# zhaoyuhsin/Edge-Guided-Near-Eye-Image-Analysis-for-Head-Mounted-Displays

Measured on AMD Instinct MI355X. Metric: eye-frames/sec (320x240): inference edge+seg (value), +fit, exact fp32, and train fwd+bwd at 1 MI355X, higher is better.
Workload: dtype f32 tensors; inference products split into f16 hi/lo pairs (3 f16 MFMAs per product, 22-bit significand), f32 accumulate (`exact_fp32`: every product on the f32 MFMA); `train`: bf16 storage, f32 accumulate, f32 master weights (and an f32-storage leg)

## Files before the change

edge-guided-near-eye-image-analysis-for-head-mounted-displays_amd/csrc/conv1x1_f16.hip:

```cpp
#include "common.h"
#include "split_f16.h"

typedef float f32x16 __attribute__((ext_vector_type(16)));
typedef float f32x4 __attribute__((ext_vector_type(4)));
typedef float f32x2 __attribute__((ext_vector_type(2)));
typedef _Float16 h8 __attribute__((ext_vector_type(8)));
typedef _Float16 h2 __attribute__((ext_vector_type(2)));
typedef unsigned u32x4 __attribute__((ext_vector_type(4)));

namespace {

constexpr unsigned OOB = 0x80000000u;

__device__ __forceinline__ __amdgpu_buffer_rsrc_t make_rsrc(const void* base, unsigned bytes) {
  return __builtin_amdgcn_make_buffer_rsrc(const_cast<void*>(base), 0, (int)bytes, 0x00020000);
}

__device__ __forceinline__ void split8(const u32x4 a, const u32x4 b, float s, h8& hi, h8& lo) {
  const f32x4 va = __builtin_bit_cast(f32x4, a), vb = __builtin_bit_cast(f32x4, b);
  const float x[8] = {va[0], va[1], va[2], va[3], vb[0], vb[1], vb[2], vb[3]};
#pragma unroll
  for (int q = 0; q < 4; ++q) {
    h2 h, l;
    egne::split2(x[2 * q], x[2 * q + 1], s, h, l);
// ... 73 lines not shown
    }
    const __amdgpu_buffer_rsrc_t ro = make_rsrc(p.out + m0 * p.out_pix_stride, (unsigned)(rows * p.out_pix_stride * 4));
    bool bad = false;
    [[maybe_unused]] int o00 = 0, o01 = 0, o10 = 0, o11 = 0;
    [[maybe_unused]] float w00 = 0.f, w01 = 0.f, w10 = 0.f, w11 = 0.f;
    [[maybe_unused]] __amdgpu_buffer_rsrc_t rres = ro;
    [[maybe_unused]] bool pix_ok = false, staged = false;
    if constexpr (UP) {
      const int ph = p.Ho, pw = p.Wo, hw = p.H * p.W;
      const long long m = m0 + li;
      pix_ok = m < M;
      const int b = pix_ok ? (int)(m / hw) : 0;
      const int r = pix_ok ? (int)(m - (long long)b * hw) : 0;
      const int y = r / p.W, x = r - y * p.W;
      float sy = 0.5f * (y + 0.5f) - 0.5f, sx = 0.5f * (x + 0.5f) - 0.5f;
      sy = sy < 0.f ? 0.f : sy; sx = sx < 0.f ? 0.f : sx;
      const int y0 = (int)sy, x0 = (int)sx, y1 = y0 + (y0 < ph - 1 ? 1 : 0), x1 = x0 + (x0 < pw - 1 ? 1 : 0);
      const float ly = sy - y0, lx = sx - x0;
      w00 = (1.f - ly) * (1.f - lx); w01 = (1.f - ly) * lx; w10 = ly * (1.f - lx); w11 = ly * lx;
      const int rs = (int)p.res_pix_stride, base = b * ph * pw;
      rres = make_rsrc(p.residual, (unsigned)((long long)p.B * ph * pw * rs * 4));
      const int r0 = (int)(m0 % hw), xb0 = r0 % p.W;
      staged = rows == 32 && xb0 + 32 <= p.W;
      if (staged) {
        const int bb = (int)(m0 / hw), yb = r0 / p.W;
        float syb = 0.5f * (yb + 0.5f) - 0.5f; syb = syb < 0.f ? 0.f : syb;
        const int yb0 = (int)syb, yb1 = yb0 + (yb0 < ph - 1 ? 1 : 0);
        const float lyb = syb - yb0;
        float sxb = 0.5f * (xb0 + 0.5f) - 0.5f; sxb = sxb < 0.f ? 0.f : sxb;
        const int cb = (int)sxb;
        constexpr int VPP = 8 * TN;
        for (int it = lane; it < UPC * VPP; it += 64) {
          const int cc = it / VPP, c4 = it - cc * VPP;
          const int gx = cb + cc < pw ? cb + cc : pw - 1;
          const int n = nt0 * 32 + c4 * 4;
          const int o0 = n < p.Cout_store ? (((bb * ph + yb0) * pw + gx) * rs + p.res_ch_off + n) * 4 : (int)OOB;
          const int o1 = n < p.Cout_store ? (((bb * ph + yb1) * pw + gx) * rs + p.res_ch_off + n) * 4 : (int)OOB;
          const f32x4 ra = __builtin_bit_cast(f32x4, __builtin_amdgcn_raw_buffer_load_b128(rres, o0, 0, 0));
          const f32x4 rb = __builtin_bit_cast(f32x4, __builtin_amdgcn_raw_buffer_load_b128(rres, o1, 0, 0));
          *(f32x4*)&patch[cc * UPP + c4 * 4] = (1.f - lyb) * ra + lyb * rb;
        }
        asm volatile("s_waitcnt vmcnt(0) lgkmcnt(0)" ::: "memory");
        o00 = ((x0 - cb) * UPP) * 4; o01 = ((x1 - cb) * UPP) * 4;
        w00 = 1.f - lx; w01 = lx;
      } else {
        o00 = ((base + y0 * pw + x0) * rs + p.res_ch_off) * 4; o01 = ((base + y0 * pw + x1) * rs + p.res_ch_off) * 4;
        o10 = ((base + y1 * pw + x0) * rs + p.res_ch_off) * 4; o11 = ((base + y1 * pw + x1) * rs + p.res_ch_off) * 4;
      }
    }
#pragma unroll
    for (int tn = 0; tn < TN; ++tn)
#pragma unroll
      for (int j = 0; j < 4; ++j) {
        const int n = (nt0 + tn) * 32 + 8 * j + 4 * kq;
        f32x4 v;
#pragma unroll
        for (int e = 0; e < 4; ++e) {
          const float t = acc[tn][4 * j + e] * out_scale + bias[tn][j][e];
          v[e] = fmaxf(t, t * slope);
        }
        if (tn == 0 && j == 0) bad |= egne_nonfinite(v[0]);
        if constexpr (UP) {
          if (staged) {
            const char* pb = (const char*)patch + (tn * 32 + 8 * j + 4 * kq) * 4;
            v += w00 * *(const f32x4*)(pb + o00) + w01 * *(const f32x4*)(pb + o01);
          } else {
          const bool on = pix_ok && n < p.Cout_store;
          const f32x4 a = __builtin_bit_cast(f32x4, __builtin_amdgcn_raw_buffer_load_b128(rres, on ? o00 + n * 4 : (int)OOB, 0, 0));
          const f32x4 b_ = __builtin_bit_cast(f32x4, __builtin_amdgcn_raw_buffer_load_b128(rres, on ? o01 + n * 4 : (int)OOB, 0, 0));
          const f32x4 c = __builtin_bit_cast(f32x4, __builtin_amdgcn_raw_buffer_load_b128(rres, on ? o10 + n * 4 : (int)OOB, 0, 0));
          const f32x4 d_ = __builtin_bit_cast(f32x4, __builtin_amdgcn_raw_buffer_load_b128(rres, on ? o11 + n * 4 : (int)OOB, 0, 0));
          v += w00 * a + w01 * b_ + w10 * c + w11 * d_;
          }
        }
        const int off = n < p.Cout_store ? (li * (int)p.out_pix_stride + p.out_ch_off + n) * 4 : (int)OOB;
        __builtin_amdgcn_raw_buffer_store_b128(__builtin_bit_cast(u32x4, v), ro, off, 0, 0);
      }
    egne_ovf_commit(bad, p.ovf_flag);
  }
}


template <int TN, bool STATS = false>
__global__ __launch_bounds__(256) void conv1x1_pool_f16x3_kernel(const egne_conv_desc p, const _Float16* __restrict__ fhi,
                                                                 const _Float16* __restrict__ flo, float a_scale, float out_scale,
                                                                 int G, long long M, int nblocks) {
  extern __shared__ __attribute__((aligned(16))) _Float16 wl[];
  const int tid = threadIdx.x, lane = tid & 63, wave = tid >> 6;
  const int li = lane & 31, kq = lane >> 5;
  const int NT = p.CoutP >> 5, nt0 = blockIdx.y * TN;
  for (int it = tid; it < G * TN * 2 * 64; it += 256) {
    const int l = it & 63, hl = (it >> 6) & 1;
    const int tn = (it >> 7) % TN, g = (it >> 7) / TN;
    const _Float16* src = (hl ? flo : fhi) + (((long long)g * NT + nt0 + tn) * 64 + l) * 8;
    *(u32x4*)&wl[(long long)it * 8] = *(const u32x4*)src;
  }
  __syncthreads();

  const float slope = p.act == EGNE_ACT_RELU ? 0.f : (p.act == EGNE_ACT_LEAKY ? 0.01f : 1.f);
  [[maybe_unused]] f32x4 bias[STATS ? 1 : TN][4];
  if constexpr (!STATS) {
#pragma unroll
  for (int tn = 0; tn < TN; ++tn)
#pragma unroll
    for (int j = 0; j < 4; ++j) {
      const int n = (nt0 + tn) * 32 + 8 * j + 4 * kq;
      bias[tn][j] = (p.bias && n < p.Cout_store) ? *(const f32x4*)(p.bias + n) : (f32x4)(0.f);
    }
  }
  const int H = p.H, W = p.W, Hp = p.Ho, Wp = p.Wo, hwp = Hp * Wp;
  const float s4 = 0.25f * a_scale;

  constexpr bool stats = STATS;
  const int bpf = (hwp + 31) >> 5, cb = stats ? (bpf + p.stats_nchunk - 1) / p.stats_nchunk : 1;
  constexpr int PP = 36;
  [[maybe_unused]] float* const patch = (float*)(wl + (long long)G * TN * 2 * 64 * 8) + wave * (32 * PP);
  [[maybe_unused]] const int rd = (lane >> 5) * PP + (lane & 31);

  for (int unit = blockIdx.x * 4 + wave; unit < nblocks; unit += gridDim.x * 4) {
   long long mfirst = (long long)unit * 32, mend = M;
   if (stats) {
     const int fb = unit / p.stats_nchunk, ck = unit - fb * p.stats_nchunk;
     mfirst = (long long)fb * hwp + (long long)ck * cb * 32;
     mend = (long long)(fb + 1) * hwp;
   }
   if (mend > mfirst + (long long)cb * 32) mend = mfirst + (long long)cb * 32;
   [[maybe_unused]] double ssum[TN], qsum[TN];
#pragma unroll
   for (int tn = 0; tn < TN; ++tn) ssum[tn] = qsum[tn] = 0.;
   for (long long m0 = mfirst; m0 < mend; m0 += 32) {
    const long long rows = mend - m0 < 32 ? mend - m0 : 32;
    const int b0 = (int)(m0 / hwp);
    const long long m = m0 + li;
    const bool valid = li < rows;
    const int b = valid ? (int)(m / hwp) : b0;
    const int r = (int)(m - (long long)b * hwp);
    const int yp = valid ? r / Wp : 0, xp = valid ? r - yp * Wp : 0;
    const int pin = ((b - b0) * H + 2 * yp) * W + 2 * xp;
    f32x16 acc[TN];
#pragma unroll
    for (int tn = 0; tn < TN; ++tn) acc[tn] = (f32x16)(0.f);
    int g = 0;
    for (int s = 0; s < p.nseg; ++s) {
      const egne_seg sg = p.seg[s];
      const long long frame = (long long)H * W * sg.pix_stride;
      const long long left = ((long long)p.B - b0) * frame * 4;
      const __amdgpu_buffer_rsrc_t rs = make_rsrc(sg.ptr + (long long)b0 * frame, (unsigned)(left < 2 * frame * 4 ? left : 2 * frame * 4));
      const int ps4 = (int)sg.pix_stride * 4;
      const int voff = valid ? (pin * (int)sg.pix_stride + sg.ch_off + 4 * kq) * 4 : (int)OOB;
      const float slope_in = sg.act_in == EGNE_ACT_RELU ? 0.f : (sg.act_in == EGNE_ACT_LEAKY ? 0.01f : 1.f);
      const float* tsc = sg.scale + (long long)b * sg.Cp + 4 * kq;
      const float* tsh = sg.shift + (long long)b * sg.Cp + 4 * kq;
      const int n16 = (sg.Cp + 15) >> 4;
      const bool tail8 = (sg.Cp & 15) != 0;
      for (int gg = 0; gg < n16; ++gg) {
        const bool has_b = !(tail8 && gg == n16 - 1);
        const int ob = has_b ? voff + 32 : (int)OOB;
        u32x4 xa[4], xb[4];
#pragma unroll
        for (int t = 0; t < 4; ++t) {
          const int d = ((t >> 1) * W + (t & 1)) * ps4;
          xa[t] = __builtin_amdgcn_raw_buffer_load_b128(rs, voff == (int)OOB ? (int)OOB : voff + d, gg * 64, 0);
          xb[t] = __builtin_amdgcn_raw_buffer_load_b128(rs, ob == (int)OOB ? (int)OOB : ob + d, gg * 64, 0);
        }
        const f32x4 sca = *(const f32x4*)(tsc + gg * 16), sha = *(const f32x4*)(tsh + gg * 16);
        const f32x4 scb = has_b ? *(const f32x4*)(tsc + gg * 16 + 8) : (f32x4)(0.f), shb = has_b ? *(const f32x4*)(tsh + gg * 16 + 8) : (f32x4)(0.f);
        f32x4 sa = (f32x4)(0.f), sb = (f32x4)(0.f);
#pragma unroll
        for (int t = 0; t < 4; ++t) {
          f32x4 va = __builtin_bit_cast(f32x4, xa[t]) * sca + sha, vb = __builtin_bit_cast(f32x4, xb[t]) * scb + shb;
#pragma unroll
          for (int e = 0; e < 4; ++e) { sa[e] += fmaxf(va[e], va[e] * slope_in); sb[e] += fmaxf(vb[e], vb[e] * slope_in); }
        }
        if (!valid) { sa = (f32x4)(0.f); sb = (f32x4)(0.f); }
        h8 ah, al;
        split8(__builtin_bit_cast(u32x4, sa), __builtin_bit_cast(u32x4, sb), s4, ah, al);
        const _Float16* wp = wl + ((long long)(g + gg) * TN * 2 * 64 + lane) * 8;
#pragma unroll
        for (int tn = 0; tn < TN; ++tn) {
          const h8 wh = *(const h8*)(wp + (tn * 2 + 0) * 512), wo = *(const h8*)(wp + (tn * 2 + 1) * 512);
          acc[tn] = __builtin_amdgcn_mfma_f32_32x32x16_f16(wh, al, acc[tn], 0, 0, 0);
          acc[tn] = __builtin_amdgcn_mfma_f32_32x32x16_f16(wo, ah, acc[tn], 0, 0, 0);
          acc[tn] = __builtin_amdgcn_mfma_f32_32x32x16_f16(wh, ah, acc[tn], 0, 0, 0);
        }
      }
      g += n16;
    }
    const __amdgpu_buffer_rsrc_t ro = make_rsrc(p.out + m0 * p.out_pix_stride, (unsigned)(rows * p.out_pix_stride * 4));
    bool bad = false;
#pragma unroll
    for (int tn = 0; tn < TN; ++tn)
#pragma unroll
      for (int j = 0; j < 4; ++j) {
        const int n = (nt0 + tn) * 32 + 8 * j + 4 * kq;
        f32x4 v, bv;
        if constexpr (STATS) bv = (p.bias && n < p.Cout_store) ? *(const f32x4*)(p.bias + n) : (f32x4)(0.f);
        else bv = bias[tn][j];
#pragma unroll
        for (int e = 0; e < 4; ++e) {
          const float t = acc[tn][4 * j + e] * out_scale + bv[e];
          v[e] = fmaxf(t, t * slope);
        }
        if (tn == 0 && j == 0) bad |= egne_nonfinite(v[0]);
        const int off = n < p.Cout_store ? (li * (int)p.out_pix_stride + p.out_ch_off + n) * 4 : (int)OOB;
        __builtin_amdgcn_raw_buffer_store_b128(__builtin_bit_cast(u32x4, v), ro, off, 0, 0);
        if constexpr (stats) {
          *(f32x4*)&patch[li * PP + 8 * j + 4 * kq] = valid ? v : (f32x4)(0.f);
          if (j == 3) {
            asm volatile("s_waitcnt lgkmcnt(0)" ::: "memory");
            double s_ = ssum[tn], q_ = qsum[tn];
#pragma unroll
            for (int i = 0; i < 16; ++i) {
              const double x = (double)patch[i * 2 * PP + rd];
              s_ += x; q_ += x * x;
            }
            ssum[tn] = s_; qsum[tn] = q_;
          }
        }
      }
    egne_ovf_commit(bad, p.ovf_flag);
   }
   if constexpr (stats) {
#pragma unroll
     for (int tn = 0; tn < TN; ++tn) {
       const double s_ = ssum[tn] + __shfl_xor(ssum[tn], 32), q_ = qsum[tn] + __shfl_xor(qsum[tn], 32);
       const int n = (nt0 + tn) * 32 + lane;
       if (lane < 32 && n < p.Cout_store)
         ((double2*)p.stats_ws)[(long long)unit * p.Cout_store + n] = make_double2(s_, q_);
     }
   }
  }
}

__global__ void pack_w1x1_f16_k(const float* __restrict__ w, int Cout, int Cin, const int* __restrict__ kmap, int G, int CoutP,
                                float wscale, _Float16* __restrict__ hi, _Float16* __restrict__ lo) {
  const long long total = (long long)G * CoutP * 16;
  const int NT = CoutP >> 5;
  for (long long i = (long long)blockIdx.x * blockDim.x + threadIdx.x; i < total; i += (long long)gridDim.x * blockDim.x) {
    const int j = (int)(i & 7), nn = (int)((i >> 3) & 31), h = (int)((i >> 8) & 1);
    long long q = i >> 9;
    const int nt = (int)(q % NT);
    const int g = (int)(q / NT);
    const int n = nt * 32 + nn, ci = kmap[g * 16 + h * 8 + j];
    const float v = (n < Cout && ci >= 0) ? w[(long long)n * Cin + ci] * wscale : 0.f;
    const _Float16 hh = (_Float16)v;
    hi[i] = hh;
    lo[i] = (_Float16)(v - (float)hh);
  }
}

}

extern "C" int egne_pack_conv1x1_weight_f16(const float* w_oihw, int Cout, int Cin, const int32_t* kmap, int G, int CoutP,
                                            float wscale, void* fhi, void* flo, void* stream) {
  EGNE_REQUIRE(w_oihw && kmap && fhi && flo && Cout > 0 && Cin > 0 && G > 0 && CoutP >= Cout && CoutP % 32 == 0 && wscale > 0.f,
               "pack_conv1x1_f16: bad sizes Cout %d Cin %d G %d CoutP %d", Cout, Cin, G, CoutP);
  long long total = (long long)G * CoutP * 16, g = (total + 255) / 256;
  if (g > 4096) g = 4096;
  hipLaunchKernelGGL(pack_w1x1_f16_k, dim3((unsigned)g), dim3(256), 0, (hipStream_t)stream, w_oihw, Cout, Cin, kmap, G, CoutP, wscale,
                     (_Float16*)fhi, (_Float16*)flo);
  return egne::check_launch("egne_pack_conv1x1_weight_f16");
}

extern "C" int egne_conv1x1_f16x3_fwd(const egne_conv_desc* dp, const void* fhi, const void* flo, float a_scale, float w_scale,
                                      void* stream) {
  EGNE_REQUIRE(dp && fhi && flo, "conv1x1_f16: null pointer");
  const egne_conv_desc& d = *dp;
  EGNE_REQUIRE(egne::fp32_storage(d), "conv1x1_f16: split-pair / f16 storage (presplit, out_split) is not known here");
  const bool up = d.residual && d.Ho * 2 == d.H && d.Wo * 2 == d.W;
  EGNE_REQUIRE(d.kh == 1 && d.kw == 1 && d.stride == 1 && d.pad_h == 0 && d.pad_w == 0 && d.ngroups == 1 && (up || (d.Ho == d.H && d.Wo == d.W)) &&
               d.nseg >= 1 && d.nseg <= EGNE_MAXSEG && (up || !d.residual) && !d.post_scale, "conv1x1_f16: unsupported descriptor");
  EGNE_REQUIRE(!up || (d.act == EGNE_ACT_NONE && ((uintptr_t)d.residual & 15) == 0 && d.res_pix_stride % 4 == 0 && d.res_ch_off % 4 == 0 &&
                       d.res_ch_off + d.Cout_store <= d.res_pix_stride && (long long)d.B * d.Ho * d.Wo * d.res_pix_stride * 4 < (1ll << 31) &&
                       (long long)d.B * d.H * d.W < (1ll << 31)),
               "conv1x1_f16: up-sampled addend (no activation, 16-byte aligned channel vectors, < 2 GB)");
  EGNE_REQUIRE(d.CoutP % 32 == 0 && (d.CoutP == 32 || d.CoutP % 64 == 0) && d.Cout_store <= d.CoutP && d.Cout_store % 4 == 0 && d.out &&
               ((uintptr_t)d.out & 15) == 0 && d.out_pix_stride % 4 == 0 && d.out_ch_off % 4 == 0 &&
               d.out_ch_off + d.Cout_store <= d.out_pix_stride, "conv1x1_f16: output");
  EGNE_REQUIRE(!d.bias || ((uintptr_t)d.bias & 15) == 0, "conv1x1_f16: bias alignment");
  int G = 0;
  for (int s = 0; s < d.nseg; ++s) {
    const egne_seg& g = d.seg[s];
    EGNE_REQUIRE(g.ptr && !g.scale && !g.shift && g.act_in == EGNE_ACT_NONE && g.Cp % 8 == 0 && g.ch_off % 4 == 0 &&
                 g.pix_stride % 4 == 0 && ((uintptr_t)g.ptr & 15) == 0 && g.ch_off + g.Cp <= g.pix_stride && g.pix_stride * 128 < (1ll << 31),
                 "conv1x1_f16: slice %d", s);
    G += (g.Cp + 15) / 16;
  }
  EGNE_REQUIRE(d.out_pix_stride * 128 < (1ll << 31) && ((uintptr_t)fhi & 15) == 0 && ((uintptr_t)flo & 15) == 0 && a_scale > 0.f && w_scale > 0.f,
               "conv1x1_f16: strides / weights / scales");
  const long long M = (long long)d.B * d.H * d.W;
  const long long nb = (M + 31) / 32;
  EGNE_REQUIRE(nb < (1ll << 31), "conv1x1_f16: too many pixels");
  const int TN = d.CoutP == 32 ? 1 : 2;
  const size_t lds = (size_t)G * TN * 2 * 64 * 8 * sizeof(_Float16);
  EGNE_REQUIRE(lds <= 80 * 1024, "conv1x1_f16: K = %d groups of 16 does not fit the LDS weight image", G);
  static bool once = [] {
    return hipFuncSetAttribute((const void*)conv1x1_f16x3_kernel<1>, hipFuncAttributeMaxDynamicSharedMemorySize, 80 * 1024) == hipSuccess &&
           hipFuncSetAttribute((const void*)conv1x1_f16x3_kernel<2>, hipFuncAttributeMaxDynamicSharedMemorySize, 80 * 1024) == hipSuccess;
  }();
  if (!once) return egne::fail(EGNE_ERR_LAUNCH, "conv1x1_f16: cannot raise the dynamic LDS limit");
  const int ny = d.CoutP / (32 * TN);
  long long gx = (nb + 3) / 4;
  const long long cap = 256 * 8;
  if (gx > cap) gx = cap;
  const float os = 1.0f / (a_scale * w_scale);
  hipStream_t st = (hipStream_t)stream;
  if (up) {
    const size_t lds_up = lds + (size_t)4 * 18 * (32 * TN + 8) * sizeof(float);
    EGNE_REQUIRE(lds_up <= 80 * 1024, "conv1x1_f16: K = %d groups of 16 leaves no room for the addend patches", G);
    static bool once_up = [] {
      return hipFuncSetAttribute((const void*)conv1x1_f16x3_kernel<1, true>, hipFuncAttributeMaxDynamicSharedMemorySize, 80 * 1024) == hipSuccess &&
             hipFuncSetAttribute((const void*)conv1x1_f16x3_kernel<2, true>, hipFuncAttributeMaxDynamicSharedMemorySize, 80 * 1024) == hipSuccess;
    }();
    if (!once_up) return egne::fail(EGNE_ERR_LAUNCH, "conv1x1_f16: cannot raise the dynamic LDS limit");
    if (TN == 1)
      hipLaunchKernelGGL((conv1x1_f16x3_kernel<1, true>), dim3((unsigned)gx, ny), dim3(256), lds_up, st, d, (const _Float16*)fhi, (const _Float16*)flo,
                         a_scale, os, G, M, (int)nb);
    else
      hipLaunchKernelGGL((conv1x1_f16x3_kernel<2, true>), dim3((unsigned)gx, ny), dim3(256), lds_up, st, d, (const _Float16*)fhi, (const _Float16*)flo,
                         a_scale, os, G, M, (int)nb);
  } else if (TN == 1)
    hipLaunchKernelGGL((conv1x1_f16x3_kernel<1>), dim3((unsigned)gx, ny), dim3(256), lds, st, d, (const _Float16*)fhi, (const _Float16*)flo,
                       a_scale, os, G, M, (int)nb);
  else
    hipLaunchKernelGGL((conv1x1_f16x3_kernel<2>), dim3((unsigned)gx, ny), dim3(256), lds, st, d, (const _Float16*)fhi, (const _Float16*)flo,
                       a_scale, os, G, M, (int)nb);
  return egne::check_launch("egne_conv1x1_f16x3_fwd");
}

extern "C" int egne_conv1x1_pool2_f16x3_fwd(const egne_conv_desc* dp, const void* fhi, const void* flo, float a_scale, float w_scale,
                                            void* stream) {
  EGNE_REQUIRE(dp && fhi && flo, "conv1x1_pool2_f16: null pointer");
  const egne_conv_desc& d = *dp;
  EGNE_REQUIRE(egne::fp32_storage(d), "conv1x1_f16: split-pair / f16 storage (presplit, out_split) is not known here");
  EGNE_REQUIRE(d.kh == 1 && d.kw == 1 && d.stride == 1 && d.pad_h == 0 && d.pad_w == 0 && d.ngroups == 1 && d.Ho == d.H / 2 && d.Wo == d.W / 2 &&
               d.Ho > 0 && d.Wo > 0 && d.nseg >= 1 && d.nseg <= EGNE_MAXSEG && !d.residual && !d.post_scale, "conv1x1_pool2_f16: unsupported descriptor");
  EGNE_REQUIRE(d.CoutP % 32 == 0 && d.CoutP <= 96 && d.Cout_store <= d.CoutP && d.Cout_store % 4 == 0 && d.out &&
               ((uintptr_t)d.out & 15) == 0 && d.out_pix_stride % 4 == 0 && d.out_ch_off % 4 == 0 &&
               d.out_ch_off + d.Cout_store <= d.out_pix_stride && (!d.bias || ((uintptr_t)d.bias & 15) == 0), "conv1x1_pool2_f16: output");
  int G = 0;
  for (int s = 0; s < d.nseg; ++s) {
    const egne_seg& g = d.seg[s];
    EGNE_REQUIRE(g.ptr && g.scale && g.shift && ((uintptr_t)g.scale & 15) == 0 && ((uintptr_t)g.shift & 15) == 0 && g.Cp % 8 == 0 &&
                 g.ch_off % 4 == 0 && g.pix_stride % 4 == 0 && ((uintptr_t)g.ptr & 15) == 0 && g.ch_off + g.Cp <= g.pix_stride &&
                 (long long)d.H * d.W * g.pix_stride * 8 < (1ll << 31), "conv1x1_pool2_f16: slice %d", s);
    G += (g.Cp + 15) / 16;
  }
  EGNE_REQUIRE(d.out_pix_stride * 128 < (1ll << 31) && ((uintptr_t)fhi & 15) == 0 && ((uintptr_t)flo & 15) == 0 && a_scale > 0.f && w_scale > 0.f,
               "conv1x1_pool2_f16: strides / weights / scales");
  const long long M = (long long)d.B * d.Ho * d.Wo;
  const long long nb = (M + 31) / 32;
  EGNE_REQUIRE(nb < (1ll << 31), "conv1x1_pool2_f16: too many pixels");
  const int TN = d.CoutP / 32;
  const int bpf = (d.Ho * d.Wo + 31) / 32;
  EGNE_REQUIRE(!d.stats_ws || (((uintptr_t)d.stats_ws & 15) == 0 && d.stats_nchunk >= 1 && d.stats_nchunk <= bpf &&
                               (long long)(d.stats_nchunk - 1) * ((bpf + d.stats_nchunk - 1) / d.stats_nchunk) < bpf &&
                               (long long)d.B * d.stats_nchunk < (1ll << 31)),
               "conv1x1_pool2_f16: stats_ws needs 1 <= stats_nchunk <= %d blocks per frame, no empty chunk", bpf);
  const size_t lds = (size_t)G * TN * 2 * 64 * 8 * sizeof(_Float16) + (d.stats_ws ? (size_t)4 * 32 * 36 * sizeof(float) : 0);
  EGNE_REQUIRE(lds <= 80 * 1024, "conv1x1_pool2_f16: K = %d groups of 16 does not fit the LDS weight image", G);
  static bool once = [] {
    return hipFuncSetAttribute((const void*)conv1x1_pool_f16x3_kernel<1>, hipFuncAttributeMaxDynamicSharedMemorySize, 80 * 1024) == hipSuccess &&
           hipFuncSetAttribute((const void*)conv1x1_pool_f16x3_kernel<2>, hipFuncAttributeMaxDynamicSharedMemorySize, 80 * 1024) == hipSuccess &&
           hipFuncSetAttribute((const void*)conv1x1_pool_f16x3_kernel<3>, hipFuncAttributeMaxDynamicSharedMemorySize, 80 * 1024) == hipSuccess &&
           hipFuncSetAttribute((const void*)conv1x1_pool_f16x3_kernel<1, true>, hipFuncAttributeMaxDynamicSharedMemorySize, 80 * 1024) == hipSuccess &&
           hipFuncSetAttribute((const void*)conv1x1_pool_f16x3_kernel<2, true>, hipFuncAttributeMaxDynamicSharedMemorySize, 80 * 1024) == hipSuccess &&
           hipFuncSetAttribute((const void*)conv1x1_pool_f16x3_kernel<3, true>, hipFuncAttributeMaxDynamicSharedMemorySize, 80 * 1024) == hipSuccess;
  }();
  if (!once) return egne::fail(EGNE_ERR_LAUNCH, "conv1x1_pool2_f16: cannot raise the dynamic LDS limit");
  const int ny = 1;
  const long long nu = d.stats_ws ? (long long)d.B * d.stats_nchunk : nb;
  long long gx = (nu + 3) / 4;
  const long long cap = 256 * 8;
  if (gx > cap) gx = cap;
  const float os = 1.0f / (a_scale * w_scale);
  hipStream_t st = (hipStream_t)stream;
  const dim3 grid((unsigned)gx, (unsigned)ny);
  const _Float16* h = (const _Float16*)fhi;
  const _Float16* l = (const _Float16*)flo;
  if (d.stats_ws) {
    if (TN == 1) hipLaunchKernelGGL((conv1x1_pool_f16x3_kernel<1, true>), grid, dim3(256), lds, st, d, h, l, a_scale, os, G, M, (int)nu);
    else if (TN == 2) hipLaunchKernelGGL((conv1x1_pool_f16x3_kernel<2, true>), grid, dim3(256), lds, st, d, h, l, a_scale, os, G, M, (int)nu);
    else hipLaunchKernelGGL((conv1x1_pool_f16x3_kernel<3, true>), grid, dim3(256), lds, st, d, h, l, a_scale, os, G, M, (int)nu);
  } else if (TN == 1) hipLaunchKernelGGL((conv1x1_pool_f16x3_kernel<1>), grid, dim3(256), lds, st, d, h, l, a_scale, os, G, M, (int)nu);
  else if (TN == 2) hipLaunchKernelGGL((conv1x1_pool_f16x3_kernel<2>), grid, dim3(256), lds, st, d, h, l, a_scale, os, G, M, (int)nu);
  else hipLaunchKernelGGL((conv1x1_pool_f16x3_kernel<3>), grid, dim3(256), lds, st, d, h, l, a_scale, os, G, M, (int)nu);
  return egne::check_launch("egne_conv1x1_pool2_f16x3_fwd");
}
```

edge-guided-near-eye-image-analysis-for-head-mounted-displays_amd/engine.py:

```python
import ctypes as C

import torch

from . import _lib
from ._lib import ACT_LEAKY, ACT_NONE, ACT_RELU


import os

HALO_ENABLED = os.environ.get("EGNE_HALO", "1") != "0"
F16X3_ENABLED = os.environ.get("EGNE_F16X3", "1") != "0"
HALO_F16_MAX_COUTP = int(os.environ.get("EGNE_HALO_F16_MAX_COUTP", "256"))
LATTICE_ENABLED = os.environ.get("EGNE_LATTICE", "1") != "0"
LAYER_BYTES = {}
TDPOOL_FUSED = os.environ.get("EGNE_TDPOOL_FUSED", "1") != "0"
TDPOOL_STATS_UNITS = 32768
HALO_POOL = os.environ.get("EGNE_HALO_POOL", "1") != "0"
POOL_FUSED = os.environ.get("EGNE_POOL_FUSED", "1") != "0"
RW_MIN_W = int(os.environ.get("EGNE_RW_MIN_W", "120"))
RW_MAX_COUTP = int(os.environ.get("EGNE_RW_MAX_COUTP", "32"))
RW_MAX_CP = int(os.environ.get("EGNE_RW_MAX_CP", "512"))
RW_ENABLED = os.environ.get("EGNE_RW", "1") != "0"
RS_ENABLED = os.environ.get("EGNE_RS", "1") != "0"
RS_MIN_W = int(os.environ.get("EGNE_RS_MIN_W", "60"))
# ... 1413 lines not shown
        d.act = layer.act
        if layer.post is not None:
            d.post_scale, d.post_shift = layer.post[0].data_ptr(), layer.post[1].data_ptr()
        if residual is not None:
            d.residual, d.res_pix_stride, d.res_ch_off = residual.ptr, residual.stride, residual.off
        d.out, d.out_pix_stride, d.out_ch_off = dst.ptr, dst.stride, dst.off
        d.Cout_store = min(layer.Cout_store, dst.Cp)
        assert tuple(dst.buf.shape[1:3]) == (Ho, Wo), (name, tuple(dst.buf.shape), Ho, Wo)
        assert dst.buf.dtype == torch.bfloat16 and all(p.buf.dtype == torch.bfloat16 for p in pieces), name
        self.keep.append(d)
        flops = 2.0 * B * Ho * Wo * layer.Cout * layer.Cin * layer.kh * layer.kw
        db = None
        if self.train:
            db = _lib.ConvDesc()
            C.memmove(C.byref(db), C.byref(d), C.sizeof(_lib.ConvDesc))
            db.Ktot, db.CoutP = layer.Ktot, layer.CoutP
            self.keep.append(db)
        ws_stats, want_partials = None, bool(getattr(self, "_want_partials", False))
        self._want_partials, self.last_partials = False, None
        if (stats or want_partials) and fast3 and STATS_FUSED and STATS_FUSED_BF16 and self.train:
            nchunk_s = ((W + 31) // 32) * ((H + 7) // 8) * 4
            ws_stats = self._stats_ws(d, B, nchunk_s)
            if want_partials:
                self.last_partials = (ws_stats, nchunk_s, int(d.Cout_store))
        if up_add is not None:
            P, ph, pw = up_add
            assert (2 * ph, 2 * pw) == (H, W) and P.Cp >= int(d.Cout_store) and tuple(P.buf.shape[:3]) == (B, ph, pw) and P.off % 8 == 0 and P.stride % 8 == 0, name
            d.Ho, d.Wo = ph, pw
            d.residual, d.res_pix_stride, d.res_ch_off = P.ptr, P.stride, P.off
        if smallcin:
            self._add(self.L.egne_conv3x3_smallcin_fwd, (C.byref(d), layer.w40.data_ptr()), name, flops=flops, kind="conv3x3_smallcin")
        elif fast3:
            self._add(self.L.egne_conv3x3_bf16_fwd, (C.byref(d), layer.bfrag.data_ptr()), name, flops=flops, kind="conv_bf16:3x3")
            self._last_b3_desc = d
        elif fast1:
            self._add(self.L.egne_conv1x1_bf16_fwd, (C.byref(d), layer.b1frag.data_ptr()), name, flops=flops, kind="conv_bf16:1x1")
        elif BF16_NARROW and int(self.L.egne_conv_narrow_bf16_supported(C.byref(d))):
            self._add(self.L.egne_conv_narrow_bf16_fwd, (C.byref(d),), name, flops=flops, kind="conv_bf16:narrow")
        else:
            self._add(self.L.egne_conv2d_fwd, (C.byref(d),), name, flops=flops, kind="conv_igemm")
        if stats:
            self.last_stats = (self._stats_finish(ws_stats, d, B, Ho * Wo, nchunk_s, name) if ws_stats is not None
                               else self.norm_stats(dst, B, Ho * Wo, name=name + ".stats")[:2])
        if self.train:
            def emit(bw, up_add=up_add):
                self._bw_conv(bw, layer, list(pieces), dst, db, B, H, W, Ho, Wo, name)
                if up_add is not None:
                    P, ph, pw = up_add
                    Pq = Piece(P.buf, P.off, min(P.C, int(db.Cout_store)), int(db.Cout_store), P.n0)
                    first = self.first_touch(Pq.buf, Pq.off, Pq.Cp, Pq.n0, B)
                    gz, gP = self.gp(dst, B), self.gp(Pq, B)
                    if first:
                        self.mark_stored(Pq, B)
                    bw.raw(self.L.egne_upsample2x_bwd_store if first else self.L.egne_upsample2x_bwd,
                           (gz.ptr, gz.stride, gz.off, gP.ptr, gP.stride, gP.off, B, ph, pw, Pq.Cp), name + ".up_add.bwd")
            self.tape.append(emit)
        return Ho, Wo

    def bf16_stream1x1_ok(self, layer, pieces, dst, B, H, W):
        if not (self.bf16 and BF16_FAST1X1 and layer.kh == 1 and layer.kw == 1 and layer.stride == 1 and layer.pad == (0, 0) and layer.post is None
                and all(p.scale is None and p.Cp % 8 == 0 and p.off % 8 == 0 and p.stride % 8 == 0 for p in pieces)
                and B * H * W >= 4096 and min(layer.Cout_store, dst.Cp) % 8 == 0 and dst.off % 8 == 0 and dst.stride % 8 == 0
                and len(pieces) <= _lib.MAXSEG):
            return False
        dq = _lib.ConvDesc()
        dq.nseg, dq.CoutP, dq.Ktot = len(pieces), layer.CoutP, layer.Ktot
        for i, p in enumerate(pieces):
            dq.seg[i].Cp = p.Cp
        return int(self.L.egne_conv1x1_bf16_pack_elems(C.byref(dq))) > 0

    def pair_fusable(self, l1, pieces, l2, dst, H, W):
        return (FUSE_1X1 and F16X3_ENABLED and not self.train and not self.bf16 and l1.split1 and l2.split and l1.kh == 1 and l1.kw == 1
                and l1.stride == 1 and l1.G == 1 and l1.pad == (0, 0) and l1.act == ACT_NONE and l1.post is None
                and all(pc.scale is None for pc in pieces) and l1.CoutP in (32, 64) and len(pieces) <= _lib.MAXSEG
                and sum((pc.Cp + 15) // 16 for pc in pieces) <= 12
                and l2.kh == 3 and l2.kw == 3 and l2.stride == 1 and l2.G == 1 and l2.pad == (1, 1) and l2.dils[0] == 1
                and l2.pad_mode == 0 and len(l2.in_layout) == 1 and l2.in_layout[0][0] == l1.Cout and l2.CoutP in (32, 64)
                and W >= FUSE_1X1_MIN_W and all(H * W * pc.stride < 2 ** 29 for pc in pieces) and H * W * dst.stride < 2 ** 29)

    def td_pool_fusable(self, layer, pieces, dst):
        G = sum((p.Cp + 15) // 16 for p in pieces)
        return (TDPOOL_FUSED and F16X3_ENABLED and not self.train and not self.bf16 and layer.split1 and layer.kh == 1 and layer.kw == 1 and layer.stride == 1
                and layer.G == 1 and layer.post is None and all(p.scale is not None for p in pieces) and len(pieces) <= _lib.MAXSEG
                and layer.CoutP <= 96 and G * (layer.CoutP // 32) * 2048 <= 80 * 1024 and dst.Cp % 4 == 0)

    def conv1x1_pooled(self, layer, pieces, dst, B, H, W, name="td", stats=False):
        assert self.td_pool_fusable(layer, pieces, dst), name
        Ho, Wo = H // 2, W // 2
        layer.need_s1 = layer.need_flat = True
        if layer not in self.layers:
            self.layers.append(layer)
        layer.ensure_packed(self.device)
        d = _lib.ConvDesc()
        d.ovf_flag, d.f16_products = self.ovf_ptr(), self.f16_products
        d.B, d.H, d.W, d.Ho, d.Wo = B, H, W, Ho, Wo
        d.kh = d.kw = d.stride = d.ngroups = 1
        d.nseg = len(pieces)
        for i, p in enumerate(pieces):
            sg = d.seg[i]
            sg.ptr, sg.pix_stride, sg.ch_off, sg.Cp = p.ptr, p.stride, p.off, p.Cp
            sg.scale, sg.shift, sg.act_in = p.scale.data_ptr(), p.shift.data_ptr(), p.act_in
        d.Ktot, d.CoutP = layer.Ktot, layer.CoutP
        d.bias = layer.bp.data_ptr() if layer.biases is not None else None
        d.act = layer.act
        d.out, d.out_pix_stride, d.out_ch_off = dst.ptr, dst.stride, dst.off
        d.Cout_store = min(layer.Cout_store, dst.Cp)
        assert tuple(dst.buf.shape[1:3]) == (Ho, Wo), (name, tuple(dst.buf.shape), Ho, Wo)
        self.keep.append(d)
        flops = 2.0 * B * Ho * Wo * layer.Cout * layer.Cin
        TN = layer.CoutP // 32
        lds = sum((p.Cp + 15) // 16 for p in pieces) * TN * 2048 + 4 * 32 * 36 * 4
        fuse_stats = stats and STATS_FUSED and dst.Cp == int(d.Cout_store) and lds <= 80 * 1024
        if fuse_stats:
            bpf = (Ho * Wo + 31) // 32
            cb = max(1, min(8, B * bpf // TDPOOL_STATS_UNITS))
            nchunk = (bpf + cb - 1) // cb
            ws = self._stats_ws(d, B, nchunk)
        self._add(self.L.egne_conv1x1_pool2_f16x3_fwd, (C.byref(d), layer.s1hi.data_ptr(), layer.s1lo.data_ptr(), F16X3_ASCALE, layer.w_scale1),
                  name, flops=flops, kind="conv_f16x3:tdpool1x1", ws=[(4, layer, "w_scale1")])
        LAYER_BYTES[name] = 4.0 * B * (H * W * sum(p.Cp for p in pieces) + Ho * Wo * int(d.Cout_store))
        if fuse_stats:
            self.last_stats = self._stats_finish(ws, d, B, Ho * Wo, nchunk, name)
        elif stats:
            self.last_stats = self.norm_stats(dst, B, Ho * Wo, name=name + ".stats")[:2]
        return Ho, Wo

    def conv_pair(self, l1, pieces, l2, dst, B, H, W, tmp=None, residual=None, name="pair", stats=False, up_add=None):
        r = self._conv_pair_impl(l1, pieces, l2, dst, B, H, W, tmp, residual, name, stats, up_add)
        LAYER_BYTES[name] = 4.0 * B * H * W * (sum(p.Cp for p in pieces) + min(l2.Cout_store, dst.Cp) + (residual.Cp if residual is not None else 0)
                                               + (8 if up_add is not None else 0))
        return r

    def _conv_pair_impl(self, l1, pieces, l2, dst, B, H, W, tmp=None, residual=None, name="pair", stats=False, up_add=None):
        fused = self.pair_fusable(l1, pieces, l2, dst, H, W)
        assert up_add is None or self.bf16 or (fused and l1.CoutP == 32 and l2.CoutP == 32 and sum((pc.Cp + 15) // 16 for pc in pieces) <= 8), name
        fused_c4 = (FUSE_1X1 and FUSE_C4 and F16X3_ENABLED and not self.train and not self.bf16 and l1.split and l2.split and l1.kh == 3 and l1.kw == 3
                    and l1.stride == 1 and l1.G == 1 and l1.pad == (1, 1) and l1.pad_mode == 0 and l1.dils[0] == 1 and l1.Cin <= 4
                    and l1.post is None and len(pieces) == 1 and pieces[0].scale is None and pieces[0].Cp >= 4 and l1.CoutP == 32
                    and l2.kh == 3 and l2.kw == 3 and l2.stride == 1 and l2.G == 1 and l2.pad == (1, 1) and l2.dils[0] == 1
                    and l2.pad_mode == 0 and len(l2.in_layout) == 1 and l2.in_layout[0][0] == l1.Cout and l2.CoutP == 32
                    and W >= FUSE_1X1_MIN_W and H * W * pieces[0].stride < 2 ** 29 and H * W * dst.stride < 2 ** 29
                    and (not isinstance(pieces[0], PlanarPiece) or l1.Cin == 1))
        assert fused_c4 or not isinstance(pieces[0], PlanarPiece), "%s: only the fused convBlock kernel reads planar inputs" % name
        if fused_c4:
            return self._conv_pair_c4(l1, pieces[0], l2, dst, B, H, W, residual, name, stats)
        if not fused:
            if tmp is None:
                tmp = Piece(self.buf(B, H, W, pad8(l1.Cout)), 0, l1.Cout)
            if (PAIR_BIAS and self.train and l1.act == ACT_NONE and l1.biases is not None and l2.biases is not None and l1.G == 1
                    and l2.G == 1 and l2.kh == 3 and l2.kw == 3 and l2.pad == (1, 1) and l2.dils[0] == 1 and l2.stride == 1
                    and l2.pad_mode == 0 and l1.Cout <= 256 and pad8(l2.Cout) <= 256 and l2.Cin == l1.Cout):
                self._pair_links[id(l1)] = l2
                self._pair_links[id(l2)] = l1
            self.conv(l1, pieces, tmp, B, H, W, name=name + ".a", up_add=up_add)
            return self.conv(l2, [tmp], dst, B, H, W, residual=residual, name=name + ".b", stats=stats)
        for p, (c, cp) in zip(pieces, l1.in_layout):
            assert p.Cp == cp and p.C == c, (name, p.C, p.Cp, c, cp)
        l1.need_s1 = True
        l1.need_flat = True
        l2.want_sfrag()
        for l in (l1, l2):
            if l not in self.layers:
                self.layers.append(l)
            l.ensure_packed(self.device)
        d1, d2 = _lib.ConvDesc(), _lib.ConvDesc()
        d2.ovf_flag, d2.f16_products = self.ovf_ptr(), self.f16_products
        for d, l in ((d1, l1), (d2, l2)):
            d.B, d.H, d.W, d.Ho, d.Wo = B, H, W, H, W
            d.kh, d.kw, d.stride = l.kh, l.kw, 1
            d.pad_h, d.pad_w, d.pad_mode, d.ngroups = l.pad[0], l.pad[1], 0, 1
            for g in range(_lib.MAXGROUP):
                d.dil[g] = 1
            d.bias = l.bp.data_ptr() if l.biases is not None else None
            d.act = l.act
        d1.nseg = len(pieces)
        for i, p in enumerate(pieces):
            sg = d1.seg[i]
            sg.ptr, sg.pix_stride, sg.ch_off, sg.Cp, sg.act_in = p.ptr, p.stride, p.off, p.Cp, ACT_NONE
        d1.Ktot, d1.CoutP = l1.Ktot, l1.CoutP
        if up_add is not None:
            P, ph, pw = up_add
            assert (2 * ph, 2 * pw) == (H, W) and P.Cp >= 32 and tuple(P.buf.shape[:3]) == (B, ph, pw)
            d1.Ho, d1.Wo = ph, pw
            d1.residual, d1.res_pix_stride, d1.res_ch_off = P.ptr, P.stride, P.off
        d2.nseg = 0
        d2.Ktot, d2.CoutP = l1.CoutP, l2.sfrag_coutp()
        if l2.post is not None:
            d2.post_scale, d2.post_shift = l2.post[0].data_ptr(), l2.post[1].data_ptr()
        if residual is not None:
            d2.residual, d2.res_pix_stride, d2.res_ch_off = residual.ptr, residual.stride, residual.off
        d2.out, d2.out_pix_stride, d2.out_ch_off = dst.ptr, dst.stride, dst.off
        d2.Cout_store = min(l2.Cout_store, dst.Cp)
        assert tuple(dst.buf.shape[1:3]) == (H, W), (name, tuple(dst.buf.shape), H, W)
        self.keep += [d1, d2]
# ... 631 lines not shown
```

Measured before the change: 2130.

## Double-buffer input loads and stage scale/shift tables in LDS for pooled 1x1 conv

```diff
diff --git a/edge-guided-near-eye-image-analysis-for-head-mounted-displays_amd/csrc/conv1x1_f16.hip b/edge-guided-near-eye-image-analysis-for-head-mounted-displays_amd/csrc/conv1x1_f16.hip
--- a/edge-guided-near-eye-image-analysis-for-head-mounted-displays_amd/csrc/conv1x1_f16.hip
+++ b/edge-guided-near-eye-image-analysis-for-head-mounted-displays_amd/csrc/conv1x1_f16.hip
@@ -179,11 +179,12 @@
 
 
 template <int TN, bool STATS = false>
-__global__ __launch_bounds__(256) void conv1x1_pool_f16x3_kernel(const egne_conv_desc p, const _Float16* __restrict__ fhi,
+__global__ __launch_bounds__(256) __attribute__((amdgpu_waves_per_eu(TN <= 2 ? 3 : 2))) void conv1x1_pool_f16x3_kernel(const egne_conv_desc p, const _Float16* __restrict__ fhi,
                                                                  const _Float16* __restrict__ flo, float a_scale, float out_scale,
                                                                  int G, long long M, int nblocks) {
   extern __shared__ __attribute__((aligned(16))) _Float16 wl[];
-  const int tid = threadIdx.x, lane = tid & 63, wave = tid >> 6;
+  const int tid = threadIdx.x, lane = tid & 63;
+  const int wave = __builtin_amdgcn_readfirstlane(tid >> 6);
   const int li = lane & 31, kq = lane >> 5;
   const int NT = p.CoutP >> 5, nt0 = blockIdx.y * TN;
   for (int it = tid; it < G * TN * 2 * 64; it += 256) {
@@ -195,8 +196,9 @@
   __syncthreads();
 
   const float slope = p.act == EGNE_ACT_RELU ? 0.f : (p.act == EGNE_ACT_LEAKY ? 0.01f : 1.f);
-  [[maybe_unused]] f32x4 bias[STATS ? 1 : TN][4];
-  if constexpr (!STATS) {
+  constexpr bool BIAS_REGS = !STATS && TN == 1;
+  [[maybe_unused]] f32x4 bias[BIAS_REGS ? TN : 1][4];
+  if constexpr (BIAS_REGS) {
 #pragma unroll
   for (int tn = 0; tn < TN; ++tn)
 #pragma unroll
@@ -213,6 +215,9 @@
   constexpr int PP = 36;
   [[maybe_unused]] float* const patch = (float*)(wl + (long long)G * TN * 2 * 64 * 8) + wave * (32 * PP);
   [[maybe_unused]] const int rd = (lane >> 5) * PP + (lane & 31);
+  constexpr int NF = STATS ? 1 : 2;
+  const int G16 = G * 16;
+  float* const tab = (float*)(wl + (long long)G * TN * 2 * 64 * 8) + (STATS ? 4 * 32 * PP : 0) + wave * (NF * 2 * G16);
 
   for (int unit = blockIdx.x * 4 + wave; unit < nblocks; unit += gridDim.x * 4) {
    long long mfirst = (long long)unit * 32, mend = M;
@@ -225,6 +230,23 @@
    [[maybe_unused]] double ssum[TN], qsum[TN];
 #pragma unroll
    for (int tn = 0; tn < TN; ++tn) ssum[tn] = qsum[tn] = 0.;
+   {
+     const int bu = (int)(mfirst / hwp);
+     int gb = 0;
+     for (int s = 0; s < p.nseg; ++s) {
+       const egne_seg sg = p.seg[s];
+       const int c16 = ((sg.Cp + 15) >> 4) * 16;
+       for (int it = lane; it < NF * c16; it += 64) {
+         const int f = it >= c16 ? 1 : 0, c = it - f * c16;
+         const bool on = c < sg.Cp && bu + f < p.B;
+         const long long at = (long long)(bu + f) * sg.Cp + c;
+         tab[(f * 2 + 0) * G16 + gb + c] = on ? sg.scale[at] : 0.f;
+         tab[(f * 2 + 1) * G16 + gb + c] = on ? sg.shift[at] : 0.f;
+       }
+       gb += c16;
+     }
+     asm volatile("s_waitcnt lgkmcnt(0)" ::: "memory");
+   }
    for (long long m0 = mfirst; m0 < mend; m0 += 32) {
     const long long rows = mend - m0 < 32 ? mend - m0 : 32;
     const int b0 = (int)(m0 / hwp);
@@ -237,51 +259,72 @@
     f32x16 acc[TN];
 #pragma unroll
     for (int tn = 0; tn < TN; ++tn) acc[tn] = (f32x16)(0.f);
-    int g = 0;
-    for (int s = 0; s < p.nseg; ++s) {
+    int is_ = 0, ig = 0, n16i = 0, ps4i = 0, voffi = (int)OOB;
+    bool tail8i = false;
+    __amdgpu_buffer_rsrc_t rsi;
+    auto open_slice = [&](int s) {
       const egne_seg sg = p.seg[s];
       const long long frame = (long long)H * W * sg.pix_stride;
       const long long left = ((long long)p.B - b0) * frame * 4;
-      const __amdgpu_buffer_rsrc_t rs = make_rsrc(sg.ptr + (long long)b0 * frame, (unsigned)(left < 2 * frame * 4 ? left : 2 * frame * 4));
-      const int ps4 = (int)sg.pix_stride * 4;
-      const int voff = valid ? (pin * (int)sg.pix_stride + sg.ch_off + 4 * kq) * 4 : (int)OOB;
-      const float slope_in = sg.act_in == EGNE_ACT_RELU ? 0.f : (sg.act_in == EGNE_ACT_LEAKY ? 0.01f : 1.f);
-      const float* tsc = sg.scale + (long long)b * sg.Cp + 4 * kq;
-      const float* tsh = sg.shift + (long long)b * sg.Cp + 4 * kq;
-      const int n16 = (sg.Cp + 15) >> 4;
-      const bool tail8 = (sg.Cp & 15) != 0;
-      for (int gg = 0; gg < n16; ++gg) {
-        const bool has_b = !(tail8 && gg == n16 - 1);
-        const int ob = has_b ? voff + 32 : (int)OOB;
-        u32x4 xa[4], xb[4];
-#pragma unroll
-        for (int t = 0; t < 4; ++t) {
-          const int d = ((t >> 1) * W + (t & 1)) * ps4;
-          xa[t] = __builtin_amdgcn_raw_buffer_load_b128(rs, voff == (int)OOB ? (int)OOB : voff + d, gg * 64, 0);
-          xb[t] = __builtin_amdgcn_raw_buffer_load_b128(rs, ob == (int)OOB ? (int)OOB : ob + d, gg * 64, 0);
-        }
-        const f32x4 sca = *(const f32x4*)(tsc + gg * 16), sha = *(const f32x4*)(tsh + gg * 16);
-        const f32x4 scb = has_b ? *(const f32x4*)(tsc + gg * 16 + 8) : (f32x4)(0.f), shb = has_b ? *(const f32x4*)(tsh + gg * 16 + 8) : (f32x4)(0.f);
-        f32x4 sa = (f32x4)(0.f), sb = (f32x4)(0.f);
-#pragma unroll
-        for (int t = 0; t < 4; ++t) {
-          f32x4 va = __builtin_bit_cast(f32x4, xa[t]) * sca + sha, vb = __builtin_bit_cast(f32x4, xb[t]) * scb + shb;
-#pragma unroll
-          for (int e = 0; e < 4; ++e) { sa[e] += fmaxf(va[e], va[e] * slope_in); sb[e] += fmaxf(vb[e], vb[e] * slope_in); }
-        }
-        if (!valid) { sa = (f32x4)(0.f); sb = (f32x4)(0.f); }
-        h8 ah, al;
-        split8(__builtin_bit_cast(u32x4, sa), __builtin_bit_cast(u32x4, sb), s4, ah, al);
-        const _Float16* wp = wl + ((long long)(g + gg) * TN * 2 * 64 + lane) * 8;
-#pragma unroll
-        for (int tn = 0; tn < TN; ++tn) {
-          const h8 wh = *(const h8*)(wp + (tn * 2 + 0) * 512), wo = *(const h8*)(wp + (tn * 2 + 1) * 512);
-          acc[tn] = __builtin_amdgcn_mfma_f32_32x32x16_f16(wh, al, acc[tn], 0, 0, 0);
-          acc[tn] = __builtin_amdgcn_mfma_f32_32x32x16_f16(wo, ah, acc[tn], 0, 0, 0);
-          acc[tn] = __builtin_amdgcn_mfma_f32_32x32x16_f16(wh, ah, acc[tn], 0, 0, 0);
-        }
-      }
-      g += n16;
+      rsi = make_rsrc(sg.ptr + (long long)b0 * frame, (unsigned)(left < 2 * frame * 4 ? left : 2 * frame * 4));
+      ps4i = (int)sg.pix_stride * 4;
+      voffi = valid ? (pin * (int)sg.pix_stride + sg.ch_off + 4 * kq) * 4 : (int)OOB;
+      n16i = (sg.Cp + 15) >> 4;
+      tail8i = (sg.Cp & 15) != 0;
+    };
+    open_slice(0);
+    auto issue = [&](u32x4 (&xa)[4], u32x4 (&xb)[4]) {
+      const bool live = is_ < p.nseg;
+      const int oa = live ? voffi : (int)OOB;
+      const int ob = (live && voffi != (int)OOB && !(tail8i && ig == n16i - 1)) ? voffi + 32 : (int)OOB;
+#pragma unroll
+      for (int t = 0; t < 4; ++t) {
+        const int d = ((t >> 1) * W + (t & 1)) * ps4i;
+        xa[t] = __builtin_amdgcn_raw_buffer_load_b128(rsi, oa, ig * 64 + d, 0);
+        xb[t] = __builtin_amdgcn_raw_buffer_load_b128(rsi, ob, ig * 64 + d, 0);
+      }
+      if (live && ++ig == n16i) {
+        ig = 0;
+        if (++is_ < p.nseg) open_slice(is_);
+      }
+    };
+    int cs = 0, cleft = (p.seg[0].Cp + 15) >> 4;
+    float slope_in = p.seg[0].act_in == EGNE_ACT_RELU ? 0.f : (p.seg[0].act_in == EGNE_ACT_LEAKY ? 0.01f : 1.f);
+    const float* const tlane = tab + (STATS ? 0 : (b - b0) * 2 * G16) + 4 * kq;
+    auto consume = [&](const u32x4 (&xa)[4], const u32x4 (&xb)[4], int k) {
+      const float* tp = tlane + k * 16;
+      const f32x4 sca = *(const f32x4*)tp, sha = *(const f32x4*)(tp + G16);
+      const f32x4 scb = *(const f32x4*)(tp + 8), shb = *(const f32x4*)(tp + G16 + 8);
+      f32x4 sa = (f32x4)(0.f), sb = (f32x4)(0.f);
+#pragma unroll
+      for (int t = 0; t < 4; ++t) {
+        f32x4 va = __builtin_bit_cast(f32x4, xa[t]) * sca + sha, vb = __builtin_bit_cast(f32x4, xb[t]) * scb + shb;
+#pragma unroll
+        for (int e = 0; e < 4; ++e) { sa[e] += fmaxf(va[e], va[e] * slope_in); sb[e] += fmaxf(vb[e], vb[e] * slope_in); }
+      }
+      if (!valid) { sa = (f32x4)(0.f); sb = (f32x4)(0.f); }
+      h8 ah, al;
+      split8(__builtin_bit_cast(u32x4, sa), __builtin_bit_cast(u32x4, sb), s4, ah, al);
+      const _Float16* wp = wl + ((long long)k * TN * 2 * 64 + lane) * 8;
+#pragma unroll
+      for (int tn = 0; tn < TN; ++tn) {
+        const h8 wh = *(const h8*)(wp + (tn * 2 + 0) * 512), wo = *(const h8*)(wp + (tn * 2 + 1) * 512);
+        acc[tn] = __builtin_amdgcn_mfma_f32_32x32x16_f16(wh, al, acc[tn], 0, 0, 0);
+        acc[tn] = __builtin_amdgcn_mfma_f32_32x32x16_f16(wo, ah, acc[tn], 0, 0, 0);
+        acc[tn] = __builtin_amdgcn_mfma_f32_32x32x16_f16(wh, ah, acc[tn], 0, 0, 0);
+      }
+      if (--cleft == 0 && ++cs < p.nseg) {
+        cleft = (p.seg[cs].Cp + 15) >> 4;
+        slope_in = p.seg[cs].act_in == EGNE_ACT_RELU ? 0.f : (p.seg[cs].act_in == EGNE_ACT_LEAKY ? 0.01f : 1.f);
+      }
+    };
+    u32x4 xa0[4], xb0[4], xa1[4], xb1[4];
+    issue(xa0, xb0);
+    for (int k = 0; k < G; k += 2) {
+      issue(xa1, xb1);
+      consume(xa0, xb0, k);
+      issue(xa0, xb0);
+      if (k + 1 < G) consume(xa1, xb1, k + 1);
     }
     const __amdgpu_buffer_rsrc_t ro = make_rsrc(p.out + m0 * p.out_pix_stride, (unsigned)(rows * p.out_pix_stride * 4));
     bool bad = false;
@@ -291,7 +334,7 @@
       for (int j = 0; j < 4; ++j) {
         const int n = (nt0 + tn) * 32 + 8 * j + 4 * kq;
         f32x4 v, bv;
-        if constexpr (STATS) bv = (p.bias && n < p.Cout_store) ? *(const f32x4*)(p.bias + n) : (f32x4)(0.f);
+        if constexpr (!BIAS_REGS) bv = (p.bias && n < p.Cout_store) ? *(const f32x4*)(p.bias + n) : (f32x4)(0.f);
         else bv = bias[tn][j];
 #pragma unroll
         for (int e = 0; e < 4; ++e) {
@@ -454,7 +497,8 @@
                                (long long)(d.stats_nchunk - 1) * ((bpf + d.stats_nchunk - 1) / d.stats_nchunk) < bpf &&
                                (long long)d.B * d.stats_nchunk < (1ll << 31)),
                "conv1x1_pool2_f16: stats_ws needs 1 <= stats_nchunk <= %d blocks per frame, no empty chunk", bpf);
-  const size_t lds = (size_t)G * TN * 2 * 64 * 8 * sizeof(_Float16) + (d.stats_ws ? (size_t)4 * 32 * 36 * sizeof(float) : 0);
+  const size_t lds = (size_t)G * TN * 2 * 64 * 8 * sizeof(_Float16) + (d.stats_ws ? (size_t)4 * 32 * 36 * sizeof(float) : 0) +
+                     (size_t)4 * (d.stats_ws ? 1 : 2) * 2 * G * 16 * sizeof(float);
   EGNE_REQUIRE(lds <= 80 * 1024, "conv1x1_pool2_f16: K = %d groups of 16 does not fit the LDS weight image", G);
   static bool once = [] {
     return hipFuncSetAttribute((const void*)conv1x1_pool_f16x3_kernel<1>, hipFuncAttributeMaxDynamicSharedMemorySize, 80 * 1024) == hipSuccess &&
diff --git a/edge-guided-near-eye-image-analysis-for-head-mounted-displays_amd/engine.py b/edge-guided-near-eye-image-analysis-for-head-mounted-displays_amd/engine.py
--- a/edge-guided-near-eye-image-analysis-for-head-mounted-displays_amd/engine.py
+++ b/edge-guided-near-eye-image-analysis-for-head-mounted-displays_amd/engine.py
@@ -1519,7 +1519,7 @@
         G = sum((p.Cp + 15) // 16 for p in pieces)
         return (TDPOOL_FUSED and F16X3_ENABLED and not self.train and not self.bf16 and layer.split1 and layer.kh == 1 and layer.kw == 1 and layer.stride == 1
                 and layer.G == 1 and layer.post is None and all(p.scale is not None for p in pieces) and len(pieces) <= _lib.MAXSEG
-                and layer.CoutP <= 96 and G * (layer.CoutP // 32) * 2048 <= 80 * 1024 and dst.Cp % 4 == 0)
+                and layer.CoutP <= 96 and G * (layer.CoutP // 32) * 2048 + G * 1024 <= 80 * 1024 and dst.Cp % 4 == 0)
 
     def conv1x1_pooled(self, layer, pieces, dst, B, H, W, name="td", stats=False):
         assert self.td_pool_fusable(layer, pieces, dst), name
@@ -1546,7 +1546,7 @@
         self.keep.append(d)
         flops = 2.0 * B * Ho * Wo * layer.Cout * layer.Cin
         TN = layer.CoutP // 32
-        lds = sum((p.Cp + 15) // 16 for p in pieces) * TN * 2048 + 4 * 32 * 36 * 4
+        lds = sum((p.Cp + 15) // 16 for p in pieces) * (TN * 2048 + 512) + 4 * 32 * 36 * 4
         fuse_stats = stats and STATS_FUSED and dst.Cp == int(d.Cout_store) and lds <= 80 * 1024
         if fuse_stats:
             bpf = (Ho * Wo + 31) // 32
```

New measurement: 2128 (median of 3 runs). About the same (-0.1%).
